# ritikasaboo13/Quantized-GEMM-for-Transformer-Inference

Measured on AMD Instinct MI355X. Metric: int8 GEMMs/sec + achieved int8-MFMA TOPS%, M=N=K=4096, 1/2/4/8 MI355X, higher is better.
Workload: dtype int8

## Files before the change

### lab/make_epi_fm.py

```python
#!/usr/bin/env python3
import os
here = os.path.dirname(os.path.abspath(__file__))
src = open(os.path.join(here, '../quantized-gemm-for-transformer-inference_amd/csrc/gemm_i8_kernels.h')).read()
a = src.index('// kNtC: the paired full-tile output stores')
b = src.index('// ------------------------------------------------------------------------------------------------\n// gemm_i8_small')
k = src[a:b]
reps = [
    ('template <int kEpi = kEpiNone, bool kI32 = false, int kSplit = kSplitNone, bool kNtC = !kI32, int kFirst64 = 30,\n'
     '          bool kBf16 = false>\n'
     '__global__ __launch_bounds__(kFmThreads, 1) void gemm_i8_fm(GemmArgs p) {',
     'template <int kMap, int kStore, int kAux, int kEpi = kEpiNone, bool kI32 = false, int kSplit = kSplitNone, bool kNtC = !kI32, int kFirst64 = 30, bool kBf16 = false>\n'
     '__global__ __launch_bounds__(kFmThreads, 1) void gemm_i8_fm_epi(GemmArgs p) {'),
    ("    group_tiles(tile, p.tiles_m, p.tiles_n, tm, tn, !outlier_epi(kEpi) && p.wide_rows ? 8 : 4);\n",
     """    if constexpr (kMap == 1 || kMap == 3) {  // XCD patches of 8 (2) tile-rows instead of 4
        constexpr int kG = kMap == 1 ? 8 : 2;
        const int per_group = kG * p.tiles_n, group = tile / per_group, first_m = group * kG;
        const int gsz = min(p.tiles_m - first_m, kG), w = tile - group * per_group;
        tm = first_m + w % gsz;
        tn = w / gsz;
    } else {
        group_tiles(tile, p.tiles_m, p.tiles_n, tm, tn);
        if (kMap == 2 && p.tiles_n % 16 == 0) tn = (tn & ~15) | ((tn & 7) << 1) | ((tn >> 3) & 1);
        if ((kMap == 4 || kMap == 5) && p.tiles_m == 8 && p.tiles_n == 64) {
            // FFN up only: XCD x (logical ids 64 x + w; w < 32 = its first round of blocks)
            const int x = tile >> 6, w = tile & 63;
            if (kMap == 4) {  // each round: all 8 tile-rows x 32 column tiles (a contiguous half of every row)
                tm = w & 7;
                tn = 32 * (w >> 5) + 4 * x + ((w >> 3) & 3);
            } else {          // each round: 4 tile-rows x all 64 column tiles (whole rows)
                tm = 4 * (w >> 5) + (w & 3);
                tn = 8 * x + ((w & 31) >> 2);
            }
        }
    }
"""),
    ("    const bool image = full && p.wide_rows;\n",
     "    const bool image = (kStore == 0 || kStore == 5) && full && p.wide_rows;\n"
     "    float lab_sink = 0.0f;\n"
     "    const auto rsC = __builtin_amdgcn_make_buffer_rsrc(p.C, 0, 0x7fffffff, 0x00020000);\n"),
    ("""#pragma unroll
            for (int np = 0; np < 4; ++np) {
                const v4f o0 = tile_out(2 * np), o1 = tile_out(2 * np + 1);""",
     """            if constexpr (kStore != 0 && kStore != 5) {
                if (full) {
                    lab_v4f q[8];
#pragma unroll
                    for (int ni = 0; ni < 8; ++ni) q[ni] = tile_out(ni);
                    if constexpr (kStore == 2) {
#pragma unroll
                        for (int ni = 0; ni < 8; ++ni) lab_sink += q[ni][0] + q[ni][1] + q[ni][2] + q[ni][3];
                    } else if constexpr (kStore == 1) {
#pragma unroll
                        for (int np = 0; np < 4; ++np) {
                            lab_v4f x1 = q[2 * np], x2 = q[2 * np + 1];
                            lab_tstage_pair<8>(x1, x2, !lo);
                            const int64_t ra = gi0 + r0 + 16 * mi + (c & 7);
                            const int jc = gj0 + c0 + 32 * np + (lo ? 0 : 16) + 4 * kq;
                            lab_store<kAux>(rsC, C, ra * p.csh + jc, x1);
                            lab_store<kAux>(rsC, C, (ra + 8) * p.csh + jc, x2);
                        }
                    } else if constexpr (kStore == 3) {
                        const int a4 = c >> 2, b4 = c & 3;
#pragma unroll
                        for (int g = 0; g < 2; ++g) {
# ... 135 lines not shown
```

### lab/make_ldsb_fm.py

```python
#!/usr/bin/env python3
import os
here = os.path.dirname(os.path.abspath(__file__))
src = open(os.path.join(here, '../quantized-gemm-for-transformer-inference_amd/csrc/gemm_i8_kernels.h')).read()
a = src.index('// kNtC: the paired full-tile output stores')
b = src.index('// ------------------------------------------------------------------------------------------------\n// gemm_i8_small')
k = src[a:b]
k = k.replace('template <int kEpi = kEpiNone, bool kI32 = false, int kSplit = kSplitNone, bool kNtC = !kI32, int kFirst64 = 30,\n'
              '          bool kBf16 = false>\n'
              '__global__ __launch_bounds__(kFmThreads, 1) void gemm_i8_fm(GemmArgs p) {',
              'template <int kKnob, int kEpi = kEpiNone, bool kI32 = false, int kSplit = kSplitNone, bool kNtC = !kI32, int kFirst64 = 30, bool kBf16 = false>\n'
              '__global__ __launch_bounds__(kFmThreads, 1) void gemm_i8_fm_ldsb(GemmArgs p) {')
loop_a = k.index('    v4i a0[8], b0[8], a1[8], b1[8], a2[8], b2[8];')
loop_b = k.index('    // the last MFMAs\' results are read by VALU below')
new_loop = r'''    v4i a0[8], b0[8], a1[8], b1[8], a2[8], b2[8];
    auto mfma = [&](v4i &acc_, const v4i &x, const v4i &y) __attribute__((always_inline)) {
        if constexpr (kKnob == 1) mfma_agpr(acc_, x, y);
        else acc_ = __builtin_amdgcn_mfma_i32_16x16x64_i8(x, y, acc_, 0, 0, 0);
    };
    if constexpr (kKnob == 0) {
        // the product's loop, builtin MFMAs
        auto ld = [&](v4i (&fa)[8], v4i (&fb)[8], int j, int u) __attribute__((always_inline)) {
            const int soff = ((j & 7) * nsub + u) * 1024;
            if (j < 8) fb[j] = __builtin_amdgcn_raw_buffer_load_b128(rsB, voff, soff, 0);
            else fa[j - 8] = __builtin_amdgcn_raw_buffer_load_b128(rsA, voff, soff, 0);
        };
        auto substep = [&](v4i (&ca)[8], v4i (&cb)[8], v4i (&na)[8], v4i (&nb)[8], int un, bool more)
                           __attribute__((always_inline)) {
            un = un < nloc ? un : nloc - 1;
            __builtin_amdgcn_s_setprio(1);
#pragma unroll
            for (int mi = 0; mi < 8; ++mi) {
#pragma unroll
                for (int ni = 0; ni < 8; ++ni) {
                    if (more && ni == 2) ld(na, nb, 2 * mi, un);
                    if (more && ni == 6) ld(na, nb, 2 * mi + 1, un);
                    mfma(acc[mi][ni], cb[ni], ca[mi]);
                }
                __builtin_amdgcn_sched_barrier(0);
            }
            __builtin_amdgcn_s_setprio(0);
        };
#pragma unroll
        for (int j = 0; j < 16; ++j) ld(a0, b0, j, 0);
        sS[tid] = sx;
        sS[BM + tid] = sw;
#pragma unroll
        for (int j = 0; j < 16; ++j) ld(a1, b1, j, nloc > 1 ? 1 : 0);
        int u = 0;
        for (; u + 3 <= nloc; u += 3) {
            substep(a0, b0, a2, b2, u + 2, true);
            substep(a1, b1, a0, b0, u + 3, true);
            substep(a2, b2, a1, b1, u + 4, true);
        }
        const int rest = nloc - u;
        if (rest > 0) {
            substep(a0, b0, a2, b2, 0, false);
            if (rest > 1) substep(a1, b1, a2, b2, 0, false);
        }
    } else {
        // B through the LDS ring: slot s at ring + 16 s KiB, half h at + 8 h KiB, fragment f at + f KiB (the image
        // area of sS: used by the epilogue only after the loop's final barrier)
        int8_t *ring = reinterpret_cast<int8_t *>(sS + 2 * BM + 4);
        // this wave's 4 fragments (4 wm .. 4 wm + 3) of B half wn, sub-step u, into ring slot `slot`: buffer LDS-DMA
# ... 84 lines not shown
```

### lab/make_stamped_fm.py

```python
#!/usr/bin/env python3
import os
here = os.path.dirname(os.path.abspath(__file__))
src = open(os.path.join(here, '../quantized-gemm-for-transformer-inference_amd/csrc/gemm_i8_kernels.h')).read()
a = src.index('// kNtC: the paired full-tile output stores')
b = src.index('// ------------------------------------------------------------------------------------------------\n// gemm_i8_small')
k = src[a:b].replace('void gemm_i8_fm(GemmArgs p)', 'void gemm_i8_fm_stamp(GemmArgs p)')

def put(s, anchor, text, after=True):
    i = s.index(anchor)
    j = i + len(anchor) if after else i
    return s[:j] + text + s[j:]

st = lambda n: f'\n    if (tid == 0) g_fm_stamp[blockIdx.x][{n}] = __builtin_amdgcn_s_memrealtime();\n'
k = put(k, '    const int voff = lane * 16;\n', st(0).lstrip('\n'))
k = put(k, '    asm volatile("s_nop 7\\n\\ts_nop 7\\n\\ts_nop 3" ::: "memory");\n', st(1).lstrip('\n') +
        '    if (tid == 0) { g_fm_stamp[blockIdx.x][4] = slice; g_fm_stamp[blockIdx.x][5] = 0; }\n')
k = put(k, '            if (tid == 0) __hip_atomic_fetch_add(p.tickets + tile, 2u, __ATOMIC_RELAXED, __HIP_MEMORY_SCOPE_AGENT);\n',
        '            if (tid == 0) { g_fm_stamp[blockIdx.x][2] = __builtin_amdgcn_s_memrealtime(); g_fm_stamp[blockIdx.x][3] = g_fm_stamp[blockIdx.x][2]; g_fm_stamp[blockIdx.x][5] = 1; }\n')
k = put(k, '    __syncthreads();  // the scale image (and the split-K hand-off above)\n', st(2).lstrip('\n'))
end = k.rstrip().rindex('}')
k = k[:end] + '''    asm volatile("s_waitcnt vmcnt(0)" ::: "memory");
    __syncthreads();
    if (tid == 0) g_fm_stamp[blockIdx.x][3] = __builtin_amdgcn_s_memrealtime();
}
'''
out = '''// gemm_fm_stamp.h -- GENERATED by lab/make_stamped_fm.py from the product gemm_i8_fm: per-block stamps (lab only).
#pragma once

#include "../quantized-gemm-for-transformer-inference_amd/csrc/gemm_i8_kernels.h"

namespace qgemm {
namespace gemm {

__device__ unsigned long long g_fm_stamp[8192][8];

''' + k + '''
}  // namespace gemm
}  // namespace qgemm
'''
open(os.path.join(here, 'gemm_fm_stamp.h'), 'w').write(out)
print('wrote lab/gemm_fm_stamp.h')
```

### lab/make_tile_fm.py

```python
#!/usr/bin/env python3
import os
here = os.path.dirname(os.path.abspath(__file__))
src = open(os.path.join(here, '../quantized-gemm-for-transformer-inference_amd/csrc/gemm_i8_kernels.h')).read()
a = src.index('// kNtC: the paired full-tile output stores')
b = src.index('// ------------------------------------------------------------------------------------------------\n// gemm_i8_small')
k = src[a:b]
reps = [
    ('template <int kEpi = kEpiNone, bool kI32 = false, int kSplit = kSplitNone, bool kNtC = !kI32, int kFirst64 = 30,\n'
     '          bool kBf16 = false>\n'
     '__global__ __launch_bounds__(kFmThreads, 1) void gemm_i8_fm(GemmArgs p) {',
     'template <int kTM, int kTN, int kGM, int kEpi = kEpiNone, bool kI32 = false, int kSplit = kSplitNone, bool kNtC = !kI32,\n'
     '          int kFirst64 = 30, bool kBf16 = false>\n'
     '__global__ __launch_bounds__(kFmThreads, 1) void gemm_i8_fm_tile(GemmArgs p) {\n'
     '    static_assert(kTM * kTN == 256 * 256 && kTM >= 128 && kTN >= 128 && kTM <= 512 && kTN <= 512, "four 128 x 128 wave tiles");\n'
     '    constexpr int kScl = 1024;  // Cx at [0, 512), Cw at [512, 1024)'),
    ('    __shared__ __attribute__((aligned(16))) float sS[2 * BM + 4 + 4 * 64 * TS + kOutlierStage];\n'
     '    float *const sO = sS + 2 * BM + 4 + 4 * 64 * TS;',
     '    __shared__ __attribute__((aligned(16))) float sS[kScl + 4 + 4 * 64 * TS + kOutlierStage];\n'
     '    float *const sO = sS + kScl + 4 + 4 * 64 * TS;'),
    ('    const int wm = wave >> 1, wn = wave & 1;',
     '    constexpr int kWC = kTN / 128;  // wave columns\n'
     '    const int wm = wave / kWC, wn = wave % kWC;'),
    ('    group_tiles(tile, p.tiles_m, p.tiles_n, tm, tn, !outlier_epi(kEpi) && p.wide_rows ? 8 : 4);',
     '    group_tiles(tile, p.tiles_m, p.tiles_n, tm, tn, kGM);'),
    ('p.A + (((int64_t)tm * 16 + wm * 8) * nsub + u0) * 1024', 'p.A + (((int64_t)tm * (kTM / 16) + wm * 8) * nsub + u0) * 1024'),
    ('p.B + (((int64_t)tn * 16 + wn * 8) * nsub + u0) * 1024', 'p.B + (((int64_t)tn * (kTN / 16) + wn * 8) * nsub + u0) * 1024'),
    ('    const int gi0 = tm * BM, gj0 = tn * BN;', '    const int gi0 = tm * kTM, gj0 = tn * kTN;'),
    ('    const float sx = kI32 ? 0.0f : p.Cx[gi0 + tid], sw = kI32 ? 0.0f : p.Cw[gj0 + tid];',
     '    float sxv[2], swv[2];\n'
     '#pragma unroll\n'
     '    for (int j = 0; j < 2; ++j) {\n'
     '        sxv[j] = !kI32 && tid + 256 * j < kTM ? p.Cx[gi0 + tid + 256 * j] : 0.0f;\n'
     '        swv[j] = !kI32 && tid + 256 * j < kTN ? p.Cw[gj0 + tid + 256 * j] : 0.0f;\n'
     '    }'),
    ('    sS[tid] = sx;\n    sS[BM + tid] = sw;',
     '#pragma unroll\n'
     '    for (int j = 0; j < 2; ++j) {\n'
     '        if (tid + 256 * j < kTM) sS[tid + 256 * j] = sxv[j];\n'
     '        if (tid + 256 * j < kTN) sS[512 + tid + 256 * j] = swv[j];\n'
     '    }'),
    ('unsigned *last = reinterpret_cast<unsigned *>(sS + 2 * BM);', 'unsigned *last = reinterpret_cast<unsigned *>(sS + kScl);'),
    ('sS + BM + c0 + 16 * ni + 4 * kq', 'sS + 512 + c0 + 16 * ni + 4 * kq'),
    ('sS[BM + c0 + ni * 16 + c]', 'sS[512 + c0 + ni * 16 + c]'),
    ('gj0 + BN <= p.n && gi0 + BM <= p.m', 'gj0 + kTN <= p.n && gi0 + kTM <= p.m'),
    ('    float *T = sS + 2 * BM + 4 + wave * 64 * TS;', '    float *T = sS + kScl + 4 + wave * 64 * TS;'),
]
for x, y in reps:
    assert x in k, 'product kernel changed: update make_tile_fm.py (' + x[:60] + ')'
    k = k.replace(x, y)
import re
left = [l for l in k.split('\n') if re.search(r'\b(BM|BN)\b', l.split('//')[0]) and 'OS = BM + 16' not in l]
assert not left, 'a BM / BN left in the copy: ' + repr(left)
out = '''// gemm_fm_tile.h -- GENERATED by lab/make_tile_fm.py from the product gemm_i8_fm: workgroup tile shapes (lab).
#pragma once

#include "../quantized-gemm-for-transformer-inference_amd/csrc/gemm_i8_kernels.h"

namespace qgemm {
namespace gemm {

''' + k + '''
}  // namespace gemm
}  // namespace qgemm
'''
open(os.path.join(here, 'gemm_fm_tile.h'), 'w').write(out)
print('wrote lab/gemm_fm_tile.h')
```

### lab/make_variant_fm.py

```python
#!/usr/bin/env python3
import os
here = os.path.dirname(os.path.abspath(__file__))
src = open(os.path.join(here, '../quantized-gemm-for-transformer-inference_amd/csrc/gemm_i8_kernels.h')).read()
a = src.index('// kNtC: the paired full-tile output stores')
b = src.index('// ------------------------------------------------------------------------------------------------\n// gemm_i8_small')
k = src[a:b]
k = k.replace('template <int kEpi = kEpiNone, bool kI32 = false, int kSplit = kSplitNone, bool kNtC = !kI32, int kFirst64 = 30,\n'
              '          bool kBf16 = false>\n'
              '__global__ __launch_bounds__(kFmThreads, 1) void gemm_i8_fm(GemmArgs p) {',
              'template <int kKnob, int kEpi = kEpiNone, bool kI32 = false, int kSplit = kSplitNone, bool kNtC = !kI32, int kFirst64 = 30, bool kBf16 = false>\n'
              '__global__ __launch_bounds__(kFmThreads, 1) void gemm_i8_fm_var(GemmArgs p) {')
reps = [
    ("        __builtin_amdgcn_s_setprio(1);\n", "        if constexpr (kKnob != 1) __builtin_amdgcn_s_setprio(1);\n"),
    ("        __builtin_amdgcn_s_setprio(0);\n    };", "        if constexpr (kKnob != 1) __builtin_amdgcn_s_setprio(0);\n    };"),
    ("            __builtin_amdgcn_sched_barrier(0);\n        }", "            if constexpr (kKnob != 2) __builtin_amdgcn_sched_barrier(0);\n        }"),
    ("""                if (more && ni == 2) ld(na, nb, 2 * mi, un);
                if (more && ni == 6) ld(na, nb, 2 * mi + 1, un);""",
     """                constexpr int P = kKnob >= 10 ? kKnob - 10 : 2;
                // kKnob 3: j -> A fragment j / 2 when j is even, B fragment j / 2 when odd (ld takes B for j < 8)
                if (more && ni == P) ld(na, nb, kKnob == 3 ? ((2 * mi) & 1 ? (2 * mi) >> 1 : 8 + ((2 * mi) >> 1)) : 2 * mi, un);
                if (more && ni == P + 4) ld(na, nb, kKnob == 3 ? ((2 * mi + 1) & 1 ? (2 * mi + 1) >> 1 : 8 + ((2 * mi + 1) >> 1)) : 2 * mi + 1, un);"""),
]
reps.append(("    group_tiles(tile, p.tiles_m, p.tiles_n, tm, tn, !outlier_epi(kEpi) && p.wide_rows ? 8 : 4);\n",
             """    if constexpr (kKnob == 4 || kKnob == 5) {  // XCD patches of 8 (4) tile-rows instead of 4
        constexpr int kG = kKnob == 4 ? 8 : 2;
        const int per_group = kG * p.tiles_n, group = tile / per_group, first_m = group * kG;
        const int gsz = min(p.tiles_m - first_m, kG), w = tile - group * per_group;
        tm = first_m + w % gsz;
        tn = w / gsz;
    } else {
        group_tiles(tile, p.tiles_m, p.tiles_n, tm, tn);
    }
"""))
reps.append(("                mfma_agpr(acc[mi][ni], cb[ni], ca[mi]);\n",
             "                if constexpr (kKnob == 6) mfma_agpr(acc[ni][mi], cb[mi], ca[ni]);\n"
             "                else mfma_agpr(acc[mi][ni], cb[ni], ca[mi]);\n"))
for x, y in reps:
    assert x in k, 'product loop changed: update make_variant_fm.py (' + x[:40] + ')'
    k = k.replace(x, y)
out = '''// gemm_fm_var.h -- GENERATED by lab/make_variant_fm.py from the product gemm_i8_fm: main-loop scheduling knobs.
#pragma once

#include "../quantized-gemm-for-transformer-inference_amd/csrc/gemm_i8_kernels.h"

namespace qgemm {
namespace gemm {

''' + k + '''
}  // namespace gemm
}  // namespace qgemm
'''
open(os.path.join(here, 'gemm_fm_var.h'), 'w').write(out)
print('wrote lab/gemm_fm_var.h')
```

### quantized-gemm-for-transformer-inference_amd/csrc/gemm_i8.hip

```cpp
#include <hip/hip_ext.h>

#include <type_traits>

#include "gemm_i8_kernels.h"

namespace qgemm {

using namespace gemm;

const char *gemm_config_name() { return "i8mfma16x16x64_t256x256_w4_wt128x128_fragmajor_direct_agpr"; }

static thread_local GemmEvents t_events;
static int g_event_mode = 0;
void set_gemm_event_mode(int mode) { g_event_mode = mode; }
void set_gemm_events(hipEvent_t start, hipEvent_t stop) { t_events = GemmEvents{start, stop}; }
GemmEvents take_gemm_events() {
    GemmEvents e = t_events;
    t_events = GemmEvents{};
    return e;
}

static bool shape_ok(const PackedView &a, const PackedView &b) {
    return a.k_pad == b.k_pad && a.rows_pad % BM == 0 && b.rows_pad % BN == 0 && a.k_pad % BK == 0;
}

struct GemmPlan {
    int tile;
    int tiles_m, tiles_n;
    int splits;
};

static GemmPlan gemm_plan(int m, int n, int k) {
    GemmPlan g{256, (int)(round_up(m, 256) / 256), (int)(round_up(n, 256) / 256), 1};
    if (m <= 0 || n <= 0 || k <= 0) return g;
    const int nk = (int)(round_up(k, BK) / BK);
    int64_t tiles = (int64_t)g.tiles_m * g.tiles_n;
    if (tiles >= 128) {
        if (tiles >= 160) return g;
        int sp = (int)(256 / tiles);
        sp = sp < nk / 8 ? sp : nk / 8;
        sp = sp < 8 ? sp : 8;
        g.splits = sp > 1 ? sp : 1;
        return g;
    }
    g = GemmPlan{64, (int)(round_up(m, 64) / 64), (int)(round_up(n, 64) / 64), 1};
    tiles = (int64_t)g.tiles_m * g.tiles_n;
    if (tiles < 256) {
        const GemmPlan g32{32, (int)(round_up(m, 32) / 32), (int)(round_up(n, 32) / 32), 1};
        const int64_t tiles32 = (int64_t)g32.tiles_m * g32.tiles_n;
        if (tiles32 >= 512 || (tiles32 >= 256 && k <= 2048)) return g32;
    }
    int sp = tiles >= 512 ? 1 : (int)(512 / tiles);
    sp = sp < nk / 16 ? sp : nk / 16;
    sp = sp < 4 ? sp : 4;
    g.splits = sp > 1 ? sp : 1;
    return g;
}

int gemm_splits(int m, int n, int k) { return gemm_plan(m, n, k).splits; }

int gemm_plan_info(int m, int n, int k, int *tile, const char **kernel) {
    const GemmPlan g = gemm_plan(m, n, k);
    if (tile) *tile = g.tile;
    if (kernel) {
        if (g.tile == 32) *kernel = "gemm_i8_small<32> (32x32 tiles, 4 waves of 16x16, 4-stage LDS-DMA ring)";
        else if (g.tile == 64)
            *kernel = g.splits > 1 ? "gemm_i8_small<64> (64x64 tiles, LDS-DMA ring, split-K)"
                                   : "gemm_i8_small<64> (64x64 tiles, LDS-DMA ring)";
        else
            *kernel = g.splits > 1 ? "gemm_i8_fm<split-K> (256x256 tiles, 4 waves of 128x128, fragment-major operands "
                                     "straight to VGPRs, AGPR accumulators, ticket-first split-K: one int32 slab per tile)"
                                   : "gemm_i8_fm (256x256 tiles, 4 waves of 128x128, fragment-major operands straight to "
                                     "VGPRs, AGPR accumulators, fused dequant epilogue)";
    }
    return g.splits;
}

constexpr size_t kTicketBytes = 4096;

size_t gemm_ticket_bytes(int m, int n, int k) { return gemm_plan(m, n, k).splits > 1 ? kTicketBytes : 0; }

size_t gemm_scratch_bytes(int m, int n, int k) {
    const GemmPlan g = gemm_plan(m, n, k);
    if (g.splits <= 1) return 0;
    const int64_t tiles = (int64_t)g.tiles_m * g.tiles_n;
    const int slabs = g.tile == 256 ? 1 : g.splits;
    return kTicketBytes + (size_t)tiles * slabs * g.tile * g.tile * 4;
}

__global__ __launch_bounds__(256) void zero_tickets_kernel(unsigned *__restrict__ t, int n) {
    const int i = blockIdx.x * 256 + threadIdx.x;
    if (i < n) t[i] = 0u;
}

template <typename Launch>
static hipError_t launch_timed(dim3 grid, dim3 block, hipStream_t stream, const GemmArgs &p, Launch kernel) {
    const GemmEvents ev = take_gemm_events();
    if ((ev.start || ev.stop) && g_event_mode == 0) {
        hipExtLaunchKernelGGL(kernel, grid, block, 0, stream, ev.start, ev.stop, 0, p);
        return hipGetLastError();
    }
    if (ev.start) (void)hipEventRecord(ev.start, stream);
    kernel<<<grid, block, 0, stream>>>(p);
    hipError_t e = hipGetLastError();
    if (ev.stop) (void)hipEventRecord(ev.stop, stream);
    return e;
}

template <int kEpi, bool kBf16 = false>
static hipError_t launch_fm(const GemmArgs &p, dim3 grid, hipStream_t stream) {
    if constexpr (!outlier_epi(kEpi)) {
        if (p.splits == 2)
            return launch_timed(grid, dim3(kFmThreads), stream, p, gemm_i8_fm<kEpi, false, kSplitFirst, true, 31, kBf16>);
        if (p.splits > 2) return hipErrorNotSupported;
    }
    return launch_timed(grid, dim3(kFmThreads), stream, p, gemm_i8_fm<kEpi, false, kSplitNone, true, 30, kBf16>);
}

template <int TB, int kEpi, int kDepth, bool kBf16 = false>
static hipError_t launch_small(const GemmArgs &p, dim3 grid, hipStream_t stream) {
    return launch_timed(grid, dim3(SmallTile<TB, kDepth>::kThreads), stream, p, gemm_i8_small<TB, kEpi, kDepth, kBf16>);
}

template <typename F>
static hipError_t with_epilogue(const float *bias, bool relu, F f) {
    if (!bias) return f(std::integral_constant<int, kEpiNone>());
    return relu ? f(std::integral_constant<int, kEpiBiasRelu>()) : f(std::integral_constant<int, kEpiBias>());
}

template <bool kBf16>
static hipError_t dispatch_dequant(const GemmPlan &g, const GemmArgs &p, dim3 grid, int64_t tiles, const float *bias,
                                   bool relu, hipStream_t stream) {
    return with_epilogue(bias, relu, [&](auto epi) {
        constexpr int kEpi = decltype(epi)::value;
        if (g.tile == 32) return launch_small<32, kEpi, 4, kBf16>(p, grid, stream);
        if (g.tile == 64)
            return tiles <= 512 ? launch_small<64, kEpi, 3, kBf16>(p, grid, stream)
                                : launch_small<64, kEpi, 2, kBf16>(p, grid, stream);
        return launch_fm<kEpi, kBf16>(p, grid, stream);
    });
}

constexpr int64_t kBf16WideRowsMin = 16384;

hipError_t launch_gemm_dequant(const PackedView &a, const PackedView &b, void *C, int64_t csh, int64_t csw, int m,
                               int n, float inv_r2, void *scratch, size_t scratch_bytes, hipStream_t stream,
                               const float *bias, bool relu, bool tickets_zeroed, bool c_bf16) {
    if (!shape_ok(a, b)) return hipErrorInvalidValue;
    const GemmPlan g = gemm_plan(m, n, (int)a.k_pad);
    GemmArgs p{a.q, b.q, a.scale, b.scale, C, csh, csw, m, n, a.k_pad, g.tiles_m, g.tiles_n,
               inv_r2, 1, nullptr, nullptr, bias, tickets_zeroed ? 1 : 0};
    const int64_t tiles = (int64_t)g.tiles_m * g.tiles_n;
    p.wide_rows = (csw == 1 && csh >= 16384) ? 1 : 0;
    if (c_bf16) p.wide_rows = (csw == 1 && csh >= kBf16WideRowsMin) ? 1 : 0;
    if (g.splits > 1 && scratch && scratch_bytes >= gemm_scratch_bytes(m, n, (int)a.k_pad)) {
        p.splits = g.splits;
        p.tickets = static_cast<unsigned *>(scratch);
        p.slabs = reinterpret_cast<int32_t *>(static_cast<char *>(scratch) + kTicketBytes);
        if (!tickets_zeroed) {
            const int nt = (int)(kTicketBytes / sizeof(unsigned));
            zero_tickets_kernel<<<(nt + 255) / 256, 256, 0, stream>>>(p.tickets, nt);
            hipError_t e = hipGetLastError();
            if (e != hipSuccess) return e;
        }
    }
    const dim3 grid((unsigned)(tiles * p.splits));
    return c_bf16 ? dispatch_dequant<true>(g, p, grid, tiles, bias, relu, stream)
// ... 46 lines not shown
```

### quantized-gemm-for-transformer-inference_amd/csrc/gemm_i8_kernels.h

```cpp
#pragma once

#include "qgemm_internal.h"

namespace qgemm {
namespace gemm {

typedef int v4i __attribute__((ext_vector_type(4)));

constexpr int BM = 256, BN = 256, BK = 128;

static_assert(BM == kRowPad && BN == kRowPad && BK == kKPad, "packed layout must match the macro-tile");


__device__ __forceinline__ int xcd_remap(int bid, int nwg) {
    const int xcd = bid & 7, q = nwg >> 3, r = nwg & 7;
    return (xcd < r ? xcd * (q + 1) : r * (q + 1) + (xcd - r) * q) + (bid >> 3);
}

__device__ __forceinline__ void group_tiles(int wgid, int tiles_m, int tiles_n, int &tm, int &tn, int kGroupM = 4) {
    const int per_group = kGroupM * tiles_n;
    const int group = wgid / per_group;
    const int first_m = group * kGroupM;
    const int gsz = min(tiles_m - first_m, kGroupM);
    const int w = wgid - group * per_group;
    tm = first_m + w % gsz;
    tn = w / gsz;
}

__device__ __forceinline__ void tile_coords(int bid, int nwg, int tiles_m, int tiles_n, int &tm, int &tn) {
    group_tiles(xcd_remap(bid, nwg), tiles_m, tiles_n, tm, tn);
}

struct GemmArgs {
    const int8_t *A;
    const int8_t *B;
    const float *Cx;
    const float *Cw;
    void *C;
    int64_t csh, csw;
    int m, n;
    int64_t k_pad;
    int tiles_m, tiles_n;
    float inv_r2;
    int splits;
    int32_t *slabs;
    unsigned *tickets;
    const float *bias;
    int reset_tickets;
    const float *xo;
    const float *wo;
    const int *ocount;
    int64_t wo_ld;
    int wide_rows;
// ... 17 lines not shown
    return o;
}

template <int MI, int NI, int kWaves>
__device__ __forceinline__ bool splitk_combine(const GemmArgs &p, unsigned *last, v4i (&acc)[MI][NI], int tile,
                                               int slice, int S, int wave, int lane, int tid) {
    constexpr int kSlabBytes = kWaves * MI * NI * 64 * 16;
    const auto rsrc = __builtin_amdgcn_make_buffer_rsrc(
        reinterpret_cast<char *>(p.slabs) + (int64_t)tile * S * kSlabBytes, 0, S * kSlabBytes, 0x00020000);
    const int lane_off = (wave * (MI * NI * 64) + lane) * 16;
#pragma unroll
    for (int mi = 0; mi < MI; ++mi)
#pragma unroll
        for (int ni = 0; ni < NI; ++ni)
            __builtin_amdgcn_raw_buffer_store_b128(acc[mi][ni], rsrc, slice * kSlabBytes + lane_off + (mi * NI + ni) * 1024,
                                                   0, 16 );
    asm volatile("s_waitcnt vmcnt(0)" ::: "memory");
    __syncthreads();
    if (tid == 0) {
        const unsigned t = __hip_atomic_fetch_add(p.tickets + tile, 1u, __ATOMIC_RELAXED, __HIP_MEMORY_SCOPE_AGENT);
        *last = t;
        if (t == (unsigned)(S - 1) && p.reset_tickets)
            __hip_atomic_store(p.tickets + tile, 0u, __ATOMIC_RELAXED, __HIP_MEMORY_SCOPE_AGENT);
    }
    __syncthreads();
    if (*last != (unsigned)(S - 1)) return false;
    __builtin_amdgcn_fence(__ATOMIC_ACQUIRE, "wavefront");
    for (int s = 0; s < S; ++s) {
        if (s == slice) continue;
#pragma unroll
        for (int mi = 0; mi < MI; ++mi)
#pragma unroll
            for (int ni = 0; ni < NI; ++ni)
                acc[mi][ni] += __builtin_amdgcn_raw_buffer_load_b128(rsrc, s * kSlabBytes + lane_off + (mi * NI + ni) * 1024,
                                                                     0, 16 );
    }
    return true;
}

__device__ __forceinline__ void mfma_agpr(v4i &acc, const v4i &a, const v4i &b) {
    asm volatile("v_mfma_i32_16x16x64_i8 %0, %1, %2, %0" : "+a"(acc) : "v"(a), "v"(b));
}

__device__ __forceinline__ const int8_t *uniform_ptr(const int8_t *q) {
    const uint64_t v = reinterpret_cast<uint64_t>(q);
    const uint32_t lo = __builtin_amdgcn_readfirstlane((uint32_t)v), hi = __builtin_amdgcn_readfirstlane((uint32_t)(v >> 32));
    return reinterpret_cast<const int8_t *>(((uint64_t)hi << 32) | lo);
}

constexpr int kFmThreads = 256;

enum SplitMode { kSplitNone = 0, kSplitFirst = 2 };

template <int kEpi = kEpiNone, bool kI32 = false, int kSplit = kSplitNone, bool kNtC = !kI32, int kFirst64 = 30,
          bool kBf16 = false>
__global__ __launch_bounds__(kFmThreads, 1) void gemm_i8_fm(GemmArgs p) {
    static_assert(!(kI32 && kEpi != kEpiNone), "raw accumulators take no epilogue extras");
    static_assert(!(kBf16 && (kI32 || outlier_epi(kEpi))), "bf16 output: the dequantized plain / bias / relu epilogues");
    static_assert(!(kI32 && kSplit), "raw accumulators are not split");
    static_assert(!(outlier_epi(kEpi) && kSplit), "the outlier epilogue runs on unsplit plans");
    constexpr int TS = 132;
    constexpr int OS = BM + 16;
    constexpr int kOutlierStage = outlier_epi(kEpi) ? 2 * 8 * OS : 0;
    __shared__ __attribute__((aligned(16))) float sS[2 * BM + 4 + 4 * 64 * TS + kOutlierStage];
    float *const sO = sS + 2 * BM + 4 + 4 * 64 * TS;
    const int tid = threadIdx.x, lane = tid & 63;
    const int wave = __builtin_amdgcn_readfirstlane(tid >> 6);
    const int wm = wave >> 1, wn = wave & 1;
    const int S = kSplit ? 2 : 1;
    const int wid = xcd_remap(blockIdx.x, gridDim.x);
    const int tile = wid / S, slice = wid - tile * S;
    int tm, tn;
    group_tiles(tile, p.tiles_m, p.tiles_n, tm, tn, !outlier_epi(kEpi) && p.wide_rows ? 8 : 4);
    const int nsub = (int)(p.k_pad / 64);
    int cut = slice * nsub / S, end = (slice + 1) * nsub / S;
    if constexpr (kSplit == kSplitFirst) {
        const int n0 = min(max(nsub * kFirst64 / 64, 1), nsub - 1);
        cut = slice ? n0 : 0;
        end = slice ? nsub : n0;
    }
    const int u0 = __builtin_amdgcn_readfirstlane(cut);
    const int nloc = __builtin_amdgcn_readfirstlane(end - cut);
    const int half_bytes = 8 * nsub * 1024 - u0 * 1024;
    const auto rsA = __builtin_amdgcn_make_buffer_rsrc(
        const_cast<int8_t *>(uniform_ptr(p.A + (((int64_t)tm * 16 + wm * 8) * nsub + u0) * 1024)), 0,
        __builtin_amdgcn_readfirstlane(half_bytes), 0x00020000);
    const auto rsB = __builtin_amdgcn_make_buffer_rsrc(
        const_cast<int8_t *>(uniform_ptr(p.B + (((int64_t)tn * 16 + wn * 8) * nsub + u0) * 1024)), 0,
        __builtin_amdgcn_readfirstlane(half_bytes), 0x00020000);
    const int voff = lane * 16;
    const int gi0 = tm * BM, gj0 = tn * BN;
    const float sx = kI32 ? 0.0f : p.Cx[gi0 + tid], sw = kI32 ? 0.0f : p.Cw[gj0 + tid];
    const int ocnt = outlier_epi(kEpi) ? __builtin_amdgcn_readfirstlane(*p.ocount) : 0;
    float oxv[8], owv[8];
    if constexpr (outlier_epi(kEpi)) {
        const int64_t i = gi0 + tid;
        const int j = gj0 + tid;
        const __attribute__((address_space(4))) int *ocs = (const __attribute__((address_space(4))) int *)p.ocols;
#pragma unroll
        for (int t = 0; t < 8; ++t) {
            const int col = t < ocnt ? ocs[t] : 0;
            oxv[t] = t < ocnt && i < p.m ? p.xo[i * p.xo_ld + col] : 0.0f;
            if constexpr (outlier_q(kEpi))
                owv[t] = t < ocnt ? (j < p.n ? dequant_w(p.B[fofs(j, col, p.k_pad)], sw) : 0.0f) : -0.0f;
            else
                owv[t] = t < ocnt ? (j < p.n ? p.wo[(int64_t)col * p.wo_ld + j] : 0.0f) : -0.0f;
        }
    }

    v4i acc[8][8];
#pragma unroll
    for (int mi = 0; mi < 8; ++mi)
#pragma unroll
        for (int ni = 0; ni < 8; ++ni) acc[mi][ni] = v4i{};
    v4i a0[8], b0[8], a1[8], b1[8], a2[8], b2[8];
    auto ld = [&](v4i (&fa)[8], v4i (&fb)[8], int j, int u) __attribute__((always_inline)) {
        const int soff = ((j & 7) * nsub + u) * 1024;
        if (j < 8) fb[j] = __builtin_amdgcn_raw_buffer_load_b128(rsB, voff, soff, 0);
        else fa[j - 8] = __builtin_amdgcn_raw_buffer_load_b128(rsA, voff, soff, 0);
    };
    auto substep = [&](v4i (&ca)[8], v4i (&cb)[8], v4i (&na)[8], v4i (&nb)[8], int un, bool more)
                       __attribute__((always_inline)) {
        un = un < nloc ? un : nloc - 1;
        __builtin_amdgcn_s_setprio(1);
#pragma unroll
        for (int mi = 0; mi < 8; ++mi) {
#pragma unroll
            for (int ni = 0; ni < 8; ++ni) {
                if (more && ni == 2) ld(na, nb, 2 * mi, un);
                if (more && ni == 6) ld(na, nb, 2 * mi + 1, un);
                mfma_agpr(acc[mi][ni], cb[ni], ca[mi]);
            }
            __builtin_amdgcn_sched_barrier(0);
        }
        __builtin_amdgcn_s_setprio(0);
    };
#pragma unroll
    for (int j = 0; j < 16; ++j) ld(a0, b0, j, 0);
    sS[tid] = sx;
    sS[BM + tid] = sw;
#pragma unroll
    for (int j = 0; j < 16; ++j) ld(a1, b1, j, nloc > 1 ? 1 : 0);
    if constexpr (outlier_epi(kEpi)) {
#pragma unroll
        for (int t = 0; t < 8; ++t) {
            sO[t * OS + tid] = oxv[t];
            sO[(8 + t) * OS + tid] = owv[t];
        }
    }
    int u = 0;
    for (; u + 3 <= nloc; u += 3) {
        substep(a0, b0, a2, b2, u + 2, true);
        substep(a1, b1, a0, b0, u + 3, true);
        substep(a2, b2, a1, b1, u + 4, true);
    }
    const int rest = nloc - u;
    if (rest > 0) {
        substep(a0, b0, a2, b2, 0, false);
        if (rest > 1) substep(a1, b1, a2, b2, 0, false);
    }
    asm volatile("s_nop 7\n\ts_nop 7\n\ts_nop 3" ::: "memory");
    if constexpr (kSplit == kSplitFirst) {
        unsigned *last = reinterpret_cast<unsigned *>(sS + 2 * BM);
        if (tid == 0) *last = __hip_atomic_fetch_add(p.tickets + tile, 1u, __ATOMIC_RELAXED, __HIP_MEMORY_SCOPE_AGENT);
        __syncthreads();
        if (*last == 0u) {
            constexpr int kSlabBytes = 4 * 8 * 8 * 64 * 16;
            const auto rs = __builtin_amdgcn_make_buffer_rsrc(reinterpret_cast<char *>(p.slabs) + (int64_t)tile * kSlabBytes,
                                                              0, kSlabBytes, 0x00020000);
            const int lane_off = (wave * 64 * 64 + lane) * 16;
#pragma unroll
            for (int mi = 0; mi < 8; ++mi)
#pragma unroll
                for (int ni = 0; ni < 8; ++ni)
                    __builtin_amdgcn_raw_buffer_store_b128(acc[mi][ni], rs, lane_off + (mi * 8 + ni) * 1024, 0, 16 );
            asm volatile("s_waitcnt vmcnt(0)" ::: "memory");
            __syncthreads();
            if (tid == 0) __hip_atomic_fetch_add(p.tickets + tile, 2u, __ATOMIC_RELAXED, __HIP_MEMORY_SCOPE_AGENT);
            return;
        }
        if (tid == 0) {
            while (__hip_atomic_load(p.tickets + tile, __ATOMIC_RELAXED, __HIP_MEMORY_SCOPE_AGENT) != 4u)
                __builtin_amdgcn_s_sleep(2);
            if (p.reset_tickets) __hip_atomic_store(p.tickets + tile, 0u, __ATOMIC_RELAXED, __HIP_MEMORY_SCOPE_AGENT);
        }
        __builtin_amdgcn_fence(__ATOMIC_ACQUIRE, "wavefront");
    }
    __syncthreads();

    const int c = lane & 15, kq = lane >> 4;
    const int r0 = wm * 128, c0 = wn * 128;
    float ox[8][2], ow[2][8];
    if constexpr (outlier_epi(kEpi)) {
#pragma unroll
        for (int tt = 0; tt < 2; ++tt) {
            const int t = 4 * tt + kq;
#pragma unroll
            for (int ni = 0; ni < 8; ++ni) ow[tt][ni] = sO[(8 + t) * OS + c0 + 16 * ni + c];
#pragma unroll
            for (int mi = 0; mi < 8; ++mi) ox[mi][tt] = sO[t * OS + r0 + 16 * mi + c];
        }
// ... 379 lines not shown
```

Measured before the change: 12220.

## Overlap epilogue stores with final k-block MFMAs via row-group finish

Adds a row-finish variant of the fm kernel for unsplit fp32 plain/bias/relu launches. The last four k-blocks are computed one 16-row group at a time, and each finished group's dequantize, DPP shuffle and store are interleaved with the next group's MFMAs. The goal is to hide the serialized epilogue, which otherwise runs after all MFMAs are done. In exchange it adds register pressure (B held for J k-blocks plus double-buffered A), more template instantiations, and a separate dispatch path for the aligned case.

```diff
diff --git a/lab/make_epi_fm.py b/lab/make_epi_fm.py
--- a/lab/make_epi_fm.py
+++ b/lab/make_epi_fm.py
@@ -7,9 +7,9 @@
 k = src[a:b]
 reps = [
     ('template <int kEpi = kEpiNone, bool kI32 = false, int kSplit = kSplitNone, bool kNtC = !kI32, int kFirst64 = 30,\n'
-     '          bool kBf16 = false>\n'
+     '          bool kBf16 = false, bool kRowFinish = false, int kRfRest = 0, bool kRfLoop = true>\n'
      '__global__ __launch_bounds__(kFmThreads, 1) void gemm_i8_fm(GemmArgs p) {',
-     'template <int kMap, int kStore, int kAux, int kEpi = kEpiNone, bool kI32 = false, int kSplit = kSplitNone, bool kNtC = !kI32, int kFirst64 = 30, bool kBf16 = false>\n'
+     'template <int kMap, int kStore, int kAux, int kEpi = kEpiNone, bool kI32 = false, int kSplit = kSplitNone, bool kNtC = !kI32, int kFirst64 = 30, bool kBf16 = false, bool kRowFinish = false, int kRfRest = 0, bool kRfLoop = true>\n'
      '__global__ __launch_bounds__(kFmThreads, 1) void gemm_i8_fm_epi(GemmArgs p) {'),
     ("    group_tiles(tile, p.tiles_m, p.tiles_n, tm, tn, !outlier_epi(kEpi) && p.wide_rows ? 8 : 4);\n",
      """    if constexpr (kMap == 1 || kMap == 3) {  // XCD patches of 8 (2) tile-rows instead of 4
diff --git a/lab/make_ldsb_fm.py b/lab/make_ldsb_fm.py
--- a/lab/make_ldsb_fm.py
+++ b/lab/make_ldsb_fm.py
@@ -6,9 +6,9 @@
 b = src.index('// ------------------------------------------------------------------------------------------------\n// gemm_i8_small')
 k = src[a:b]
 k = k.replace('template <int kEpi = kEpiNone, bool kI32 = false, int kSplit = kSplitNone, bool kNtC = !kI32, int kFirst64 = 30,\n'
-              '          bool kBf16 = false>\n'
+              '          bool kBf16 = false, bool kRowFinish = false, int kRfRest = 0, bool kRfLoop = true>\n'
               '__global__ __launch_bounds__(kFmThreads, 1) void gemm_i8_fm(GemmArgs p) {',
-              'template <int kKnob, int kEpi = kEpiNone, bool kI32 = false, int kSplit = kSplitNone, bool kNtC = !kI32, int kFirst64 = 30, bool kBf16 = false>\n'
+              'template <int kKnob, int kEpi = kEpiNone, bool kI32 = false, int kSplit = kSplitNone, bool kNtC = !kI32, int kFirst64 = 30, bool kBf16 = false, bool kRowFinish = false, int kRfRest = 0, bool kRfLoop = true>\n'
               '__global__ __launch_bounds__(kFmThreads, 1) void gemm_i8_fm_ldsb(GemmArgs p) {')
 loop_a = k.index('    v4i a0[8], b0[8], a1[8], b1[8], a2[8], b2[8];')
 loop_b = k.index('    // the last MFMAs\' results are read by VALU below')
diff --git a/lab/make_stamped_fm.py b/lab/make_stamped_fm.py
--- a/lab/make_stamped_fm.py
+++ b/lab/make_stamped_fm.py
@@ -13,8 +13,19 @@
 
 st = lambda n: f'\n    if (tid == 0) g_fm_stamp[blockIdx.x][{n}] = __builtin_amdgcn_s_memrealtime();\n'
 k = put(k, '    const int voff = lane * 16;\n', st(0).lstrip('\n'))
-k = put(k, '    asm volatile("s_nop 7\\n\\ts_nop 7\\n\\ts_nop 3" ::: "memory");\n', st(1).lstrip('\n') +
+k = put(k, '    // the last MFMAs\' results are read by VALU below; the asm statements hide them from hipcc\'s padding\n'
+        '    asm volatile("s_nop 7\\n\\ts_nop 7\\n\\ts_nop 3" ::: "memory");\n', st(1).lstrip('\n') +
         '    if (tid == 0) { g_fm_stamp[blockIdx.x][4] = slice; g_fm_stamp[blockIdx.x][5] = 0; }\n')
+rf_st = lambda n: f'if (tid == 0) g_fm_stamp[blockIdx.x][{n}] = __builtin_amdgcn_s_memrealtime();\n'
+k = put(k, '            // the last group\'s results are read by VALU next; the asm statements hide the MFMAs from hipcc\'s padding\n',
+        '            ' + rf_st(1) + '            if (tid == 0) { g_fm_stamp[blockIdx.x][2] = g_fm_stamp[blockIdx.x][1]; '
+        'g_fm_stamp[blockIdx.x][4] = slice; g_fm_stamp[blockIdx.x][5] = 0; }\n', after=False)
+k = put(k, '                    const int rl = 16 * g + (q == 6 ? 0 : 8);\n',
+        '                    if (g == 0 && np == 0 && q == 6) { ' + rf_st(6).rstrip('\n') + ' }\n')
+k = put(k, '        return;\n    }\n    int u = 0;\n',
+        '', after=False).replace('        return;\n    }\n    int u = 0;\n',
+        '        asm volatile("s_waitcnt vmcnt(0)" ::: "memory");\n        __syncthreads();\n        ' + rf_st(3) +
+        '        return;\n    }\n    int u = 0;\n', 1)
 k = put(k, '            if (tid == 0) __hip_atomic_fetch_add(p.tickets + tile, 2u, __ATOMIC_RELAXED, __HIP_MEMORY_SCOPE_AGENT);\n',
         '            if (tid == 0) { g_fm_stamp[blockIdx.x][2] = __builtin_amdgcn_s_memrealtime(); g_fm_stamp[blockIdx.x][3] = g_fm_stamp[blockIdx.x][2]; g_fm_stamp[blockIdx.x][5] = 1; }\n')
 k = put(k, '    __syncthreads();  // the scale image (and the split-K hand-off above)\n', st(2).lstrip('\n'))
diff --git a/lab/make_tile_fm.py b/lab/make_tile_fm.py
--- a/lab/make_tile_fm.py
+++ b/lab/make_tile_fm.py
@@ -7,10 +7,10 @@
 k = src[a:b]
 reps = [
     ('template <int kEpi = kEpiNone, bool kI32 = false, int kSplit = kSplitNone, bool kNtC = !kI32, int kFirst64 = 30,\n'
-     '          bool kBf16 = false>\n'
+     '          bool kBf16 = false, bool kRowFinish = false, int kRfRest = 0, bool kRfLoop = true>\n'
      '__global__ __launch_bounds__(kFmThreads, 1) void gemm_i8_fm(GemmArgs p) {',
      'template <int kTM, int kTN, int kGM, int kEpi = kEpiNone, bool kI32 = false, int kSplit = kSplitNone, bool kNtC = !kI32,\n'
-     '          int kFirst64 = 30, bool kBf16 = false>\n'
+     '          int kFirst64 = 30, bool kBf16 = false, bool kRowFinish = false, int kRfRest = 0, bool kRfLoop = true>\n'
      '__global__ __launch_bounds__(kFmThreads, 1) void gemm_i8_fm_tile(GemmArgs p) {\n'
      '    static_assert(kTM * kTN == 256 * 256 && kTM >= 128 && kTN >= 128 && kTM <= 512 && kTN <= 512, "four 128 x 128 wave tiles");\n'
      '    constexpr int kScl = 1024;  // Cx at [0, 512), Cw at [512, 1024)'),
@@ -44,6 +44,8 @@
     ('sS[BM + c0 + ni * 16 + c]', 'sS[512 + c0 + ni * 16 + c]'),
     ('gj0 + BN <= p.n && gi0 + BM <= p.m', 'gj0 + kTN <= p.n && gi0 + kTM <= p.m'),
     ('    float *T = sS + 2 * BM + 4 + wave * 64 * TS;', '    float *T = sS + kScl + 4 + wave * 64 * TS;'),
+    ('float *const sBias = sS + 2 * BM + 4;', 'float *const sBias = sS + kScl + 4;'),
+    ('const float *const sCw = sS + BM + c0 + 4 * kq;', 'const float *const sCw = sS + 512 + c0 + 4 * kq;'),
 ]
 for x, y in reps:
     assert x in k, 'product kernel changed: update make_tile_fm.py (' + x[:60] + ')'
diff --git a/lab/make_variant_fm.py b/lab/make_variant_fm.py
--- a/lab/make_variant_fm.py
+++ b/lab/make_variant_fm.py
@@ -6,9 +6,9 @@
 b = src.index('// ------------------------------------------------------------------------------------------------\n// gemm_i8_small')
 k = src[a:b]
 k = k.replace('template <int kEpi = kEpiNone, bool kI32 = false, int kSplit = kSplitNone, bool kNtC = !kI32, int kFirst64 = 30,\n'
-              '          bool kBf16 = false>\n'
+              '          bool kBf16 = false, bool kRowFinish = false, int kRfRest = 0, bool kRfLoop = true>\n'
               '__global__ __launch_bounds__(kFmThreads, 1) void gemm_i8_fm(GemmArgs p) {',
-              'template <int kKnob, int kEpi = kEpiNone, bool kI32 = false, int kSplit = kSplitNone, bool kNtC = !kI32, int kFirst64 = 30, bool kBf16 = false>\n'
+              'template <int kKnob, int kEpi = kEpiNone, bool kI32 = false, int kSplit = kSplitNone, bool kNtC = !kI32, int kFirst64 = 30, bool kBf16 = false, bool kRowFinish = false, int kRfRest = 0, bool kRfLoop = true>\n'
               '__global__ __launch_bounds__(kFmThreads, 1) void gemm_i8_fm_var(GemmArgs p) {')
 reps = [
     ("        __builtin_amdgcn_s_setprio(1);\n", "        if constexpr (kKnob != 1) __builtin_amdgcn_s_setprio(1);\n"),
diff --git a/quantized-gemm-for-transformer-inference_amd/csrc/gemm_i8.hip b/quantized-gemm-for-transformer-inference_amd/csrc/gemm_i8.hip
--- a/quantized-gemm-for-transformer-inference_amd/csrc/gemm_i8.hip
+++ b/quantized-gemm-for-transformer-inference_amd/csrc/gemm_i8.hip
@@ -67,11 +67,16 @@
         else if (g.tile == 64)
             *kernel = g.splits > 1 ? "gemm_i8_small<64> (64x64 tiles, LDS-DMA ring, split-K)"
                                    : "gemm_i8_small<64> (64x64 tiles, LDS-DMA ring)";
+        else if (g.splits > 1)
+            *kernel = "gemm_i8_fm<split-K> (256x256 tiles, 4 waves of 128x128, fragment-major operands "
+                      "straight to VGPRs, AGPR accumulators, ticket-first split-K: one int32 slab per tile)";
+        else if (round_up(k, BK) / 64 >= kRowFinishJ + 3)
+            *kernel = "gemm_i8_fm<row-finish> (256x256 tiles, 4 waves of 128x128, fragment-major operands straight to "
+                      "VGPRs, AGPR accumulators, fused dequant epilogue; the last 4 k-blocks row group by row group, "
+                      "each group's stores under the next one's MFMAs)";
         else
-            *kernel = g.splits > 1 ? "gemm_i8_fm<split-K> (256x256 tiles, 4 waves of 128x128, fragment-major operands "
-                                     "straight to VGPRs, AGPR accumulators, ticket-first split-K: one int32 slab per tile)"
-                                   : "gemm_i8_fm (256x256 tiles, 4 waves of 128x128, fragment-major operands straight to "
-                                     "VGPRs, AGPR accumulators, fused dequant epilogue)";
+            *kernel = "gemm_i8_fm (256x256 tiles, 4 waves of 128x128, fragment-major operands straight to "
+                      "VGPRs, AGPR accumulators, fused dequant epilogue)";
     }
     return g.splits;
 }
@@ -113,6 +118,19 @@
         if (p.splits == 2)
             return launch_timed(grid, dim3(kFmThreads), stream, p, gemm_i8_fm<kEpi, false, kSplitFirst, true, 31, kBf16>);
         if (p.splits > 2) return hipErrorNotSupported;
+        if constexpr (!kBf16) {
+            if (!p.wide_rows && p.csw == 1 && p.csh % 4 == 0 && (reinterpret_cast<uintptr_t>(p.C) & 15) == 0 &&
+                p.k_pad / 64 >= kRowFinishJ + 3 && p.k_pad % BK == 0)
+            {
+                const int pre = (int)(p.k_pad / 64) - kRowFinishJ - 2;
+                const int rest = pre % 3;
+                auto go = [&](auto kernel) { return launch_timed(grid, dim3(kFmThreads), stream, p, kernel); };
+                if (pre == 2) return go(gemm_i8_fm<kEpi, false, kSplitNone, true, 30, false, true, 2, false>);
+                if (rest == 0) return go(gemm_i8_fm<kEpi, false, kSplitNone, true, 30, false, true, 0, true>);
+                if (rest == 1) return go(gemm_i8_fm<kEpi, false, kSplitNone, true, 30, false, true, 1, true>);
+                return go(gemm_i8_fm<kEpi, false, kSplitNone, true, 30, false, true, 2, true>);
+            }
+        }
     }
     return launch_timed(grid, dim3(kFmThreads), stream, p, gemm_i8_fm<kEpi, false, kSplitNone, true, 30, kBf16>);
 }
diff --git a/quantized-gemm-for-transformer-inference_amd/csrc/gemm_i8_kernels.h b/quantized-gemm-for-transformer-inference_amd/csrc/gemm_i8_kernels.h
--- a/quantized-gemm-for-transformer-inference_amd/csrc/gemm_i8_kernels.h
+++ b/quantized-gemm-for-transformer-inference_amd/csrc/gemm_i8_kernels.h
@@ -1,4 +1,6 @@
 #pragma once
+
+#include <type_traits>
 
 #include "qgemm_internal.h"
 
@@ -122,10 +124,15 @@
 
 enum SplitMode { kSplitNone = 0, kSplitFirst = 2 };
 
+constexpr int kRowFinishJ = 4;
+
+
 template <int kEpi = kEpiNone, bool kI32 = false, int kSplit = kSplitNone, bool kNtC = !kI32, int kFirst64 = 30,
-          bool kBf16 = false>
+          bool kBf16 = false, bool kRowFinish = false, int kRfRest = 0, bool kRfLoop = true>
 __global__ __launch_bounds__(kFmThreads, 1) void gemm_i8_fm(GemmArgs p) {
     static_assert(!(kI32 && kEpi != kEpiNone), "raw accumulators take no epilogue extras");
+    static_assert(!(kRowFinish && (kI32 || kSplit || kBf16 || outlier_epi(kEpi) || !kNtC)),
+                  "row finish: the unsplit fp32 plain / bias / relu launches");
     static_assert(!(kBf16 && (kI32 || outlier_epi(kEpi))), "bf16 output: the dequantized plain / bias / relu epilogues");
     static_assert(!(kI32 && kSplit), "raw accumulators are not split");
     static_assert(!(outlier_epi(kEpi) && kSplit), "the outlier epilogue runs on unsplit plans");
@@ -161,6 +168,8 @@
     const int voff = lane * 16;
     const int gi0 = tm * BM, gj0 = tn * BN;
     const float sx = kI32 ? 0.0f : p.Cx[gi0 + tid], sw = kI32 ? 0.0f : p.Cw[gj0 + tid];
+    float sb = 0.0f;
+    if constexpr (kRowFinish && has_bias(kEpi)) sb = gj0 + tid < p.n ? p.bias[gj0 + tid] : 0.0f;
     const int ocnt = outlier_epi(kEpi) ? __builtin_amdgcn_readfirstlane(*p.ocount) : 0;
     float oxv[8], owv[8];
     if constexpr (outlier_epi(kEpi)) {
@@ -217,6 +226,161 @@
             sO[t * OS + tid] = oxv[t];
             sO[(8 + t) * OS + tid] = owv[t];
         }
+    }
+    if constexpr (kRowFinish) {
+        constexpr int J = kRowFinishJ;
+        typedef float v2f __attribute__((ext_vector_type(2)));
+        typedef float v4f __attribute__((ext_vector_type(4)));
+        float *const sBias = sS + 2 * BM + 4;
+        if constexpr (has_bias(kEpi)) sBias[tid] = sb;
+        asm volatile("s_waitcnt lgkmcnt(0)" ::: "memory");
+        __builtin_amdgcn_s_barrier();
+        asm volatile("" ::: "memory");
+#pragma unroll
+        for (int mi = 0; mi < 8; ++mi)
+#pragma unroll
+            for (int ni = 0; ni < 8; ++ni) asm volatile("" : "+a"(acc[mi][ni]));
+        asm volatile("s_nop 7" ::: "memory");
+        const int n1 = nloc - J;
+        const int c = lane & 15, kq = lane >> 4;
+        const int r0 = wm * 128, c0 = wn * 128;
+        const bool lo = c < 8;
+        const v2f inv2 = {p.inv_r2, p.inv_r2};
+        const v2f zero2 = {0.0f, 0.0f};
+        float *C = static_cast<float *>(p.C);
+        const bool pairs = p.csw == 1 && (p.csh % 4 == 0) && ((reinterpret_cast<uintptr_t>(p.C) & 15) == 0) &&
+                           gj0 + BN <= p.n && gi0 + BM <= p.m;
+        float *const Cl = C + (int64_t)(gi0 + r0 + (c & 7)) * p.csh + gj0 + c0 + (lo ? 0 : 16) + 4 * kq;
+        const float *const sCw = sS + BM + c0 + 4 * kq;
+        const float *const sBv = sBias + c0 + 4 * kq;
+        auto half_out = [&](v4f &o, const v4i &a, float cx, const v4f &cw, const v4f &bv, int h) __attribute__((always_inline)) {
+            const v2f x = {cx, cx};
+            const v2f s = x * v2f{cw[2 * h], cw[2 * h + 1]} + zero2;
+            const v2f d = (v2f{(float)a[2 * h], (float)a[2 * h + 1]} * s) * inv2;
+#pragma unroll
+            for (int e = 0; e < 2; ++e) {
+                float v = d[e];
+                if constexpr (has_bias(kEpi)) v = __fadd_rn(v, bv[2 * h + e]);
+                if constexpr (has_relu(kEpi)) v = (v < 0.0f) ? 0.0f : v;
+                o[2 * h + e] = v;
+            }
+        };
+        auto tail = [&](v4i (&ca)[8], v4i (&cb)[8], v4i (&na)[8], v4i (&nb)[8]) __attribute__((always_inline)) {
+            v4i Bh[J][8], Ab[2][J];
+            auto ldB = [&](int t) __attribute__((always_inline)) {
+                Bh[t >> 3][t & 7] = __builtin_amdgcn_raw_buffer_load_b128(rsB, voff, ((t & 7) * nsub + n1 + (t >> 3)) * 1024, 0);
+            };
+            auto ldA = [&](int buf, int g, int j) __attribute__((always_inline)) {
+                Ab[buf][j] = __builtin_amdgcn_raw_buffer_load_b128(rsA, voff + j * 1024, (g * nsub + n1) * 1024, 0);
+            };
+            __builtin_amdgcn_s_setprio(1);
+#pragma unroll
+            for (int mi = 0; mi < 8; ++mi) {
+#pragma unroll
+                for (int ni = 0; ni < 8; ++ni) {
+                    if (ni == 2) ldB(2 * mi);
+                    if (ni == 6) ldB(2 * mi + 1);
+                    mfma_agpr(acc[mi][ni], cb[ni], ca[mi]);
+                }
+                __builtin_amdgcn_sched_barrier(0);
+            }
+#pragma unroll
+            for (int mi = 0; mi < 8; ++mi) {
+#pragma unroll
+                for (int ni = 0; ni < 8; ++ni) {
+                    if (ni == 2) ldB(16 + 2 * mi);
+                    if (ni == 4 && mi < J) ldA(0, 0, mi);
+                    if (ni == 6) ldB(16 + 2 * mi + 1);
+                    mfma_agpr(acc[mi][ni], nb[ni], na[mi]);
+                }
+                __builtin_amdgcn_sched_barrier(0);
+            }
+            __builtin_amdgcn_s_setprio(0);
+            v4i ta, tb;
+            v4f o0, o1, w0, w1, bb0 = {}, bb1 = {};
+            float cxg = 0.0f, r0v[4], r1v[4];
+            auto piece = [&](int g, int np, int q) __attribute__((always_inline)) {
+                if (q == 0) {
+                    if (np == 0) cxg = sS[r0 + 16 * g + c];
+                    w0 = *reinterpret_cast<const v4f *>(sCw + 32 * np);
+                    w1 = *reinterpret_cast<const v4f *>(sCw + 32 * np + 16);
+                    if constexpr (has_bias(kEpi)) {
+                        bb0 = *reinterpret_cast<const v4f *>(sBv + 32 * np);
+                        bb1 = *reinterpret_cast<const v4f *>(sBv + 32 * np + 16);
+                    }
+                    asm volatile("" : "+a"(acc[g][2 * np]));
+                    asm volatile("" : "+a"(acc[g][2 * np + 1]));
+                    ta = acc[g][2 * np];
+                    tb = acc[g][2 * np + 1];
+                } else if (q <= 2) {
+                    half_out(o0, ta, cxg, w0, bb0, q - 1);
+                } else if (q <= 4) {
+                    half_out(o1, tb, cxg, w1, bb1, q - 3);
+                } else if (q == 5) {
+#pragma unroll
+                    for (int e = 0; e < 4; ++e) {
+                        r0v[e] = __int_as_float(__builtin_amdgcn_mov_dpp(__float_as_int(o0[e]), 0x128, 0xf, 0xf, false));
+                        r1v[e] = __int_as_float(__builtin_amdgcn_mov_dpp(__float_as_int(o1[e]), 0x128, 0xf, 0xf, false));
+                    }
+                } else {
+                    v4f x;
+#pragma unroll
+                    for (int e = 0; e < 4; ++e) x[e] = q == 6 ? (lo ? o0[e] : r1v[e]) : (lo ? r0v[e] : o1[e]);
+                    const int rl = 16 * g + (q == 6 ? 0 : 8);
+                    if (pairs) {
+                        __builtin_nontemporal_store(x, reinterpret_cast<v4f *>(Cl + (int64_t)rl * p.csh + 32 * np));
+                    } else {
+                        const int64_t ra = gi0 + r0 + rl + (c & 7);
+                        const int jc = gj0 + c0 + 32 * np + (lo ? 0 : 16) + 4 * kq;
+                        if (ra < p.m) {
+#pragma unroll
+                            for (int e = 0; e < 4; ++e)
+                                if (jc + e < p.n) C[ra * p.csh + (int64_t)(jc + e) * p.csw] = x[e];
+                        }
+                    }
+                }
+            };
+#pragma unroll
+            for (int g = 0; g < 8; ++g) {
+                if (g < 7) {
+#pragma unroll
+                    for (int j = 0; j < J; ++j) ldA((g + 1) & 1, g + 1, j);
+                }
+#pragma unroll
+                for (int j = 0; j < J; ++j)
+#pragma unroll
+                    for (int ni = 0; ni < 8; ++ni) {
+                        mfma_agpr(acc[g][ni], Bh[j][ni], Ab[g & 1][j]);
+                        if (g > 0) piece(g - 1, j, ni);
+                        __builtin_amdgcn_sched_barrier(0);
+                    }
+            }
+            asm volatile("s_nop 7\n\ts_nop 7\n\ts_nop 3" ::: "memory");
+#pragma unroll
+            for (int np = 0; np < 4; ++np)
+#pragma unroll
+                for (int q = 0; q < 8; ++q) piece(7, np, q);
+        };
+        int u = 0;
+        if constexpr (kRfLoop) {
+            do {
+                substep(a0, b0, a2, b2, u + 2, true);
+                substep(a1, b1, a0, b0, u + 3, true);
+                substep(a2, b2, a1, b1, u + 4, true);
+                u += 3;
+            } while (u + 3 + kRfRest <= n1 - 2);
+        }
+        if constexpr (kRfRest == 0) {
+            tail(a0, b0, a1, b1);
+        } else if constexpr (kRfRest == 1) {
+            substep(a0, b0, a2, b2, u + 2, true);
+            tail(a1, b1, a2, b2);
+        } else {
+            substep(a0, b0, a2, b2, u + 2, true);
+            substep(a1, b1, a0, b0, u + 3, true);
+            tail(a2, b2, a0, b0);
+        }
+        return;
     }
     int u = 0;
     for (; u + 3 <= nloc; u += 3) {
```

After: 12480 (median of 6 runs). +2.1%, better.
